# leosampaio/sketchformer

Hardware: AMD Instinct MI355X
Metric: stroke-tokens/sec training step, d_model=128 L=200 B=128, 1/2/4/8 GPU (higher is better)
Workload: dtype f32; 1 GPU; cfg2: sketch-transformer-tf2 4L/8H/d128/dff512 L=200 V=1004 C=345 dropout=0.1, fwd+bwd+Adam(WarmupDecay); global_batch=128, per_gpu_batch=128, seq_len=200, parallelism=dp1, hip_graph=0, dense_gemm_arithmetic=fp32 operands split exactly into 3 bf16 pieces, 6 product...

## Files before the change

### sketchformer_amd/csrc/skf_model_bwd.hip

```cpp
#include "skf_model_internal.h"

namespace skf_model_detail {
namespace {

template <typename F>
int with_ready_event(SkfModel* M, bool want, hipEvent_t* ready, F call) {
  hipEvent_t e = (want && may_park(M)) ? M->sched.take_event() : nullptr;
  bool rode = false;
  const int rc = with_tail_event(M, e, &rode, call);
  *ready = rode ? e : nullptr;
  return rc;
}

int ffn_bwd(SkfModel* M, const DenseP& f1, const DenseP& f2, const float* x_in, const float* h, const float* dy,
            float* dh, float* dx_acc, int rows, hipStream_t s, const void* hbits, const void* image_t) {
  if (M->ctx.ffn_fused) {
    SKF_TRY(dense_wgrad(M, f2, h, f2.in, dy, f2.out, rows, s));
    SKF_TRY(M->sched.before_write(M, dh, s));
    SKF_TRY(M->sched.before_write(M, dx_acc, s));
    const int* blocks = M->ctx.live_blocks(rows, 16);
    hipEvent_t ready = nullptr;
    SKF_TRY(with_ready_event(M, M->sched.holding(), &ready, [&] {
      return skf_ffn_fused_bwd_f32(rows, M->cfg.d_model, M->cfg.dff, dy, image_t, hbits, dh, dx_acc, 1, blocks, blocks ? 16 : 0,
                                   M->cfg.gemm_precision, s);
// ... 113 lines not shown
  SKF_TRY(skf_target_live_len(M->at<long long>(P.tar), Le, B, Ld, M->at<int>(P.live_len), s));
  SKF_TRY(skf_row_blocks_build(M->at<int>(P.live_len), B, Ld, 16, M->at<int>(P.live16), s));
  SKF_TRY(skf_row_blocks_build(M->at<int>(P.live_len), B, Ld, 32, M->at<int>(P.live32), s));
  M->ctx.lists_built = true;
  return SKF_OK;
}

}

int run_backward(SkfModel* M, hipStream_t s) {
  M->ctx.begin_backward();
  M->sched.begin_backward();
  M->red.begin_step();
  const SkfConfig& c = M->cfg;
  const Layout& L = M->lay;
  const Plan& P = M->plan;
  const int B = c.batch, Le = c.seq_len, Ld = c.seq_len - 1, d = c.d_model, H = c.num_heads, dh = d / H;
  const int Me = B * Le, Md = B * Ld, N = c.num_layers;
  const float rate = c.dropout_rate;
  const long long* inp = M->at<long long>(P.inp);
  const long long* tar = M->at<long long>(P.tar);
  const unsigned char* emask = M->at<unsigned char>(P.enc_mask);
  const unsigned char* dmask = M->at<unsigned char>(P.dec_mask);
  float* G = M->at<float>(P.gA);
  float* G2 = M->at<float>(P.gB);
  float* dO = M->at<float>(P.do_);
  float* dpre = M->at<float>(P.dpre);
  float* demb = M->at<float>(P.demb);
  int layer_no = 0;

  const bool bott = has_bott(c), cls = has_cls(c), recon = do_recon(c);
  float* enc_out = M->at<float>(P.enc[N - 1].x2);
  const float* pre = bott ? M->at<float>(P.pre) : enc_out;
  if (recon) {
  if (!M->ctx.lists_built) SKF_TRY(build_row_lists(M, s));
  if (M->ctx.lists_built) M->ctx.set_live(Md, M->at<int>(P.live_len), 16, M->at<int>(P.live16), 32, M->at<int>(P.live32));
  M->ctx.lists_built = false;
  const float* dlog = M->at<float>(P.logits);
  SKF_TRY(dense_wgrad(M, L.out, M->at<float>(P.dec[N - 1].out3), d, dlog, L.out.out, Md, s));
  {
    hipEvent_t ready = nullptr;
    SKF_TRY(with_ready_event(M, true, &ready, [&] { return dense_dgrad(M, L.out, dlog, L.out.out, Md, G, d, 0, nullptr, 0, s); }));
    SKF_TRY(M->sched.issue(M, s, ready));
  }
  const unsigned char* cross_mask = c.blind_decoder_mask ? nullptr : emask;
  for (int i = N - 1; i >= 0; --i, ++layer_no) {
    const DecLayerP& w = L.dec[i];
    const DecAct& a = P.dec[i];
    const Plan::GradSet& gs = P.gs[layer_no % P.n_gs];
    float* dy3 = M->at<float>(gs.dy[0]); float* dy2 = M->at<float>(gs.dy[1]); float* dy1 = M->at<float>(gs.dy[2]);
    float* dqkv = M->at<float>(gs.dqkv); float* dkv2 = M->at<float>(gs.dkv2); float* dq2 = M->at<float>(gs.dq2);
    SKF_TRY(ffn_ln_bwd(M, w.ln3, w.f1, w.f2, G, M->at<float>(a.z3), M->at<float>(a.st3), M->at<float>(a.out2), M->at<float>(a.h), dy3,
                       M->at<float>(gs.dh), G2, Md, rate, site_dec(N, i, 2), s, hbits_of(M, a.hbits, Md), M->at<char>(a.img[1])));
    SKF_TRY(ln_oproj_bwd(M, w.ln2, w.mha2.o, G2, M->at<float>(a.z2), M->at<float>(a.st2), M->at<float>(a.o2), G, dy2, dO, Md, rate,
                         site_dec(N, i, 1), s, M->at<char>(a.img_o2)));
    const float* kv2 = M->at<float>(a.kv2);
    SKF_TRY(M->sched.before_write(M, dq2, s));
    SKF_TRY(M->sched.before_write(M, dkv2, s));
    const int* qlive = M->ctx.live_lengths(Md);
    SKF_TRY(skf_attention_bwd_ordered(M->at<float>(a.q2), d, kv2, 2 * d, kv2 + d, 2 * d, M->at<float>(a.o2), d, dO, d,
                                      M->at<float>(a.astats2), cross_mask, Le, 0, B, H, Ld, Le, dh, dq2, d, dkv2, 2 * d,
                                      dkv2 + d, 2 * d, M->cfg.gemm_precision, qlive, M->ctx.order, s));
    SKF_TRY(dense_wgrad(M, w.mha2.q, M->at<float>(a.out1), d, dq2, d, Md, s));
    const bool lead = row_owner_takes_ln(M, w.ln1, ln_oproj_partial_bytes(M, Md), Md, &w.mha1.o, &w.mha2.q);
    if (!lead) SKF_TRY(dense_dgrad(M, w.mha2.q, dq2, d, Md, G, d, 1, nullptr, 0, s));
    SKF_TRY(dense_wgrad(M, w.mha2.kv, pre, L.E, dkv2, 2 * d, Me, s));
    if (i == 0) {
      SKF_TRY(M->sched.before_read(M, dpre, s));
      SKF_TRY(dense_dgrad(M, w.mha2.kv, dkv2, 2 * d, Me, dpre, L.E, i != N - 1, nullptr, 0, s));
    } else SKF_TRY(dense_dgrad_deferred(M, w.mha2.kv, dkv2, 2 * d, Me, dpre, L.E, i != N - 1, s));
    SKF_TRY(ln_oproj_bwd(M, w.ln1, w.mha1.o, G, M->at<float>(a.z1), M->at<float>(a.st1), M->at<float>(a.o1), G2, dy1, dO, Md, rate,
                         site_dec(N, i, 0), s, M->at<char>(a.img_o1), lead ? dq2 : nullptr, lead ? M->at<char>(a.img_q2t) : nullptr));
    const float* qkv = M->at<float>(a.qkv);
    SKF_TRY(M->sched.before_write(M, dqkv, s));
    SKF_TRY(skf_attention_bwd_ordered(qkv, 3 * d, qkv + d, 3 * d, qkv + 2 * d, 3 * d, M->at<float>(a.o1), d, dO, d,
                                      M->at<float>(a.astats1), dmask, Ld, 1, B, H, Ld, Ld, dh, dqkv, 3 * d, dqkv + d, 3 * d,
                                      dqkv + 2 * d, 3 * d, M->cfg.gemm_precision, qlive, M->ctx.order, s));
    SKF_TRY(dense_wgrad(M, w.mha1.qkv, M->at<float>(a.x_in), d, dqkv, 3 * d, Md, s));
    const bool hold = M->ctx.ffn_fused && i > 0;
    hipEvent_t ready = nullptr;
    SKF_TRY(with_ready_event(M, !hold, &ready, [&] { return dense_dgrad(M, w.mha1.qkv, dqkv, 3 * d, Md, G2, d, 1, nullptr, 0, s); }));
    float* t = G; G = G2; G2 = t;
    if (hold) SKF_TRY(M->sched.hold(M, s));
    else SKF_TRY(M->sched.issue(M, s, ready));
  }
  M->ctx.clear_live();
  hipEvent_t dec_emb_done = nullptr;
  if (c.continuous) {
    SKF_TRY(skf_embed_continuous_bwd(M->at<float>(P.tar), Le, B, Ld, G, d, M->G(L.dec_embd.w), M->G(L.dec_embd.b), rate,
                                     site_dec_embed(N), M->state, M->at<char>(P.small_ws), P.small_ws_bytes, s));
  } else {
    if (P.emb_sort_bytes) {
      SKF_TRY(with_ready_event(M, M->n_buckets == 2, &dec_emb_done, [&] {
        return skf_embed_bwd_sorted(M->at<char>(P.emb_sort[1]), B, Ld, G, c.vocab_size, d, M->G(L.dec_emb), rate, site_dec_embed(N), M->state, s);
      }));
    } else {
      SKF_HIP(hipMemsetAsync(M->G(L.dec_emb), 0, (size_t)c.vocab_size * d * sizeof(float), s));
      SKF_TRY(skf_embed_bwd(tar, Le, B, Ld, G, c.vocab_size, d, M->G(L.dec_emb), rate, site_dec_embed(N), M->state, s));
    }
  }
  if (M->n_buckets == 2) SKF_TRY(flush_wgrads(M, s, 0, false, true, dec_emb_done));
  SKF_TRY(M->sched.before_read(M, dpre, s));
  }
  const int E = L.E, Ua = L.Ua, U = c.lowerdim, NB = c.class_buffer_layers;
  hipEvent_t bott_ready = nullptr;
  if (bott) {
    const bool defer_sums = M->sched.side && Ua <= 4096;
    float* xp1 = M->at<float>(P.bott_part);
    float* xp2 = xp1 + (size_t)B * Le;
    float* pvp = xp2 + (size_t)B * Le;
    if (recon && defer_sums) {
      SKF_TRY(skf_expander_bwd_partials(dpre, M->at<float>(P.emb), M->P(L.exp_w), B, Le, E, demb, 0, xp1, xp2, s));
      SKF_TRY(colsum_desc(M, xp1, B, Le, M->G(L.exp_w)));
      SKF_TRY(colsum_desc(M, xp2, B, Le, M->G(L.exp_b)));
    } else if (recon)
      SKF_TRY(skf_expander_bwd(dpre, M->at<float>(P.emb), M->P(L.exp_w), B, Le, E, demb, 0, M->G(L.exp_w), M->G(L.exp_b),
                               M->at<char>(P.small_ws), P.small_ws_bytes, s));
    const int acc_emb = recon ? 1 : 0;
    const float* dcls = M->at<float>(P.cls_logits);
    if (cls && NB == 0) {
      SKF_TRY(dense_wgrad(M, L.cls, M->at<float>(P.emb), E, dcls, c.n_classes, B, s));
      SKF_TRY(dense_dgrad(M, L.cls, dcls, c.n_classes, B, demb, E, acc_emb, nullptr, 0, s));
    } else if (cls) {
      float* dz = M->at<float>(P.dcb[0]);
      float* dz2 = M->at<float>(P.dcb[1]);
      SKF_TRY(M->sched.before_write(M, dz, s));
      SKF_TRY(dense_wgrad(M, L.cls, M->at<float>(P.cb_f[NB - 1]), U, dcls, c.n_classes, B, s));
      SKF_TRY(dense_dgrad(M, L.cls, dcls, c.n_classes, B, dz, U, 0, M->at<float>(P.cb_h[NB - 1]), U, s));
      for (int i = NB - 1; i >= 0; --i) {
        SKF_TRY(skf_dropout(dz, dz, (size_t)B * U, c.class_dropout, site_class(N, i), M->state, s));
        const float* in = i == 0 ? M->at<float>(P.emb) : M->at<float>(P.cb_f[i - 1]);
        const int in_w = i == 0 ? E : U;
        SKF_TRY(dense_wgrad(M, L.cbuf[i], in, in_w, dz, U, B, s));
        if (i == 0) {
          SKF_TRY(dense_dgrad(M, L.cbuf[0], dz, U, B, demb, E, acc_emb, nullptr, 0, s));
        } else {
          SKF_TRY(M->sched.before_write(M, dz2, s));
          SKF_TRY(dense_dgrad(M, L.cbuf[i], dz, U, B, dz2, U, 0, M->at<float>(P.cb_h[i - 1]), U, s));
          float* t = dz; dz = dz2; dz2 = t;
        }
      }
    }
    const float* dpool = demb;
    if (c.attn_version == 2) {
      SKF_TRY(M->sched.before_write(M, M->at<float>(P.dpooled), s));
      SKF_TRY(dense_wgrad(M, L.bott_e, M->at<float>(P.pooled), d, demb, U, B, s));
      SKF_TRY(dense_dgrad(M, L.bott_e, demb, U, B, M->at<float>(P.dpooled), d, 0, nullptr, 0, s));
      dpool = M->at<float>(P.dpooled);
    }
    SKF_TRY(M->sched.before_write(M, G, s));
    if (defer_sums) {
      SKF_TRY(skf_pool_bwd_partials(M->at<float>(P.u), M->P(L.bott_v), enc_out, M->at<float>(P.pool_a), dpool, B, Le, Ua, d, G, pvp, s));
      SKF_TRY(colsum_desc(M, pvp, B, Ua, M->G(L.bott_v)));
    } else
    SKF_TRY(skf_pool_bwd(M->at<float>(P.u), M->P(L.bott_v), enc_out, M->at<float>(P.pool_a), dpool, B, Le, Ua, d,
                         G, M->G(L.bott_v), M->at<char>(P.small_ws), P.small_ws_bytes, s));
    SKF_TRY(dense_wgrad(M, L.bott_w, enc_out, d, M->at<float>(P.u), Ua, Me, s));
    SKF_TRY(with_ready_event(M, true, &bott_ready, [&] { return dense_dgrad(M, L.bott_w, M->at<float>(P.u), Ua, Me, G, d, 1, nullptr, 0, s); }));
  } else {
    float* spare = (G == M->at<float>(P.gA)) ? M->at<float>(P.gB) : M->at<float>(P.gA);
    G = dpre; G2 = spare;
  }
  SKF_TRY(M->sched.issue(M, s, bott_ready));
  for (int i = N - 1; i >= 0; --i, ++layer_no) {
    const EncLayerP& w = L.enc[i];
    const EncAct& a = P.enc[i];
    const Plan::GradSet& gs = P.gs[layer_no % P.n_gs];
    float* dy2 = M->at<float>(gs.dy[0]); float* dy1 = M->at<float>(gs.dy[1]);
    float* dqkv = M->at<float>(gs.dqkv);
    SKF_TRY(ffn_ln_bwd(M, w.ln2, w.f1, w.f2, G, M->at<float>(a.z2), M->at<float>(a.st2), M->at<float>(a.x1), M->at<float>(a.h), dy2,
                       M->at<float>(gs.dh), G2, Me, rate, site_enc(i, 1), s, hbits_of(M, a.hbits, Me), M->at<char>(a.img[1])));
    if (i == 0) SKF_TRY(M->sched.issue(M, s, M->ctx.last_ready));
    M->ctx.last_ready = nullptr;
    {
      hipEvent_t ready = nullptr;
      SKF_TRY(with_ready_event(M, i == 0, &ready, [&] {
        return ln_oproj_bwd(M, w.ln1, w.mha.o, G2, M->at<float>(a.z1), M->at<float>(a.st1), M->at<float>(a.o), G, dy1, dO, Me, rate,
                            site_enc(i, 0), s, M->at<char>(a.img_o));
      }));
      if (i == 0) SKF_TRY(M->sched.issue(M, s, ready));
    }
    const float* qkv = M->at<float>(a.qkv);
// ... 57 lines not shown
```

### sketchformer_amd/csrc/skf_model_fwd.hip

```cpp
#include "skf_model_internal.h"

namespace skf_model_detail {

int classify_fwd(SkfModel* M, bool training, hipStream_t s) {
  const SkfConfig& c = M->cfg;
  const Layout& L = M->lay;
  const Plan& P = M->plan;
  const float* fc = M->at<float>(P.emb);
  for (int i = 0; i < c.class_buffer_layers; ++i) {
    float* h = M->at<float>(P.cb_h[i]);
    float* fdrop = M->at<float>(P.cb_f[i]);
    SKF_TRY(dense_fwd(M, L.cbuf[i], fc, c.batch, h, 1, s));
    const float r = training ? c.class_dropout : 0.f;
    SKF_TRY(skf_dropout(h, fdrop, (size_t)c.batch * c.lowerdim, r, site_class(c.num_layers, i), M->state, s));
    fc = fdrop;
  }
  return dense_fwd(M, L.cls, fc, c.batch, M->at<float>(P.cls_logits), 0, s);
}

namespace {
bool ffn_fused_on(const SkfModel* M) {
  const SkfConfig& c = M->cfg;
  return !(M->flags & SKF_MODEL_FFN_LAUNCHES) && skf_ffn_fused_supported(c.batch * c.seq_len, c.d_model, c.dff, c.gemm_precision) &&
         skf_ffn_image_bytes(c.d_model, c.dff, c.gemm_precision) > 0;
}
int build_ffn_images(SkfModel* M, bool with_backward, bool encoder_only, hipStream_t s) {
  const SkfConfig& c = M->cfg;
  const Layout& L = M->lay;
  const Plan& P = M->plan;
  const int d = c.d_model, F = c.dff;
  const size_t half = skf_ffn_image_bytes(d, F, c.gemm_precision) / 2;
  std::vector<const float*> src; std::vector<int> ld, tr, K, N; std::vector<void*> img;
  auto one = [&](const DenseP& w, int t, int k, int n, char* im) {
    src.push_back(M->P(w.w)); ld.push_back(w.ld); tr.push_back(t); K.push_back(k); N.push_back(n); img.push_back(im);
  };
  auto ffn = [&](const DenseP& f1, const DenseP& f2, const size_t (&im)[2]) {
    one(f1, 0, d, F, M->at<char>(im[0])); one(f2, 0, F, d, M->at<char>(im[0]) + half);
    if (with_backward) { one(f2, 1, d, F, M->at<char>(im[1])); one(f1, 1, F, d, M->at<char>(im[1]) + half); }
  };
  const bool dec = !encoder_only && do_recon(c);
  for (int i = 0; i < c.num_layers; ++i) {
    ffn(L.enc[i].f1, L.enc[i].f2, P.enc[i].img);
    if (i > 0) one(L.enc[i].mha.qkv, 0, d, 3 * d, M->at<char>(P.enc[i].img_qkv));
    one(L.enc[i].mha.o, 0, d, d, M->at<char>(P.enc[i].img_of));
    if (with_backward) one(L.enc[i].mha.o, 1, d, d, M->at<char>(P.enc[i].img_o));
  }
  if (dec)
    for (int i = 0; i < c.num_layers; ++i) {
      ffn(L.dec[i].f1, L.dec[i].f2, P.dec[i].img);
      if (i > 0) one(L.dec[i].mha1.qkv, 0, d, 3 * d, M->at<char>(P.dec[i].img_qkv));
      one(L.dec[i].mha2.o, 0, d, d, M->at<char>(P.dec[i].img_o2f));
      one(L.dec[i].mha1.o, 0, d, d, M->at<char>(P.dec[i].img_o1f)); one(L.dec[i].mha2.q, 0, d, d, M->at<char>(P.dec[i].img_q2));
      if (with_backward) { one(L.dec[i].mha1.o, 1, d, d, M->at<char>(P.dec[i].img_o1)); one(L.dec[i].mha2.o, 1, d, d, M->at<char>(P.dec[i].img_o2)); }
// ... 92 lines not shown
    SKF_TRY(skf_embed_continuous_fwd(inpf, Le, B, Le, M->P(L.enc_embd.w), M->P(L.enc_embd.b), d, M->pos,
                                     M->at<float>(P.enc[0].x_in), rate, site_enc_embed(), M->state, s));
  else
    SKF_TRY(skf_embed_fwd(inp, Le, B, Le, M->P(L.enc_emb), c.vocab_size, d, M->pos, M->at<float>(P.enc[0].x_in), rate,
                          site_enc_embed(), M->state, s));
  bool enc_qkv_done = false;
  for (int i = 0; i < N; ++i) {
    const EncLayerP& w = L.enc[i];
    const EncAct& a = P.enc[i];
    float* x = M->at<float>(a.x_in);
    float* qkv = M->at<float>(a.qkv);
    if (!enc_qkv_done) SKF_TRY(dense_fwd(M, w.mha.qkv, x, Me, qkv, 0, s));
    if (i == 0 && images_ready) SKF_HIP(hipStreamWaitEvent(s, masks_ready, 0));
    SKF_TRY(skf_attention_fwd_ordered(qkv, 3 * d, qkv + d, 3 * d, qkv + 2 * d, 3 * d, emask, Le, 0, B, H, Le, Le, dh,
                                      M->at<float>(a.o), d, M->at<float>(a.astats), M->cfg.gemm_precision, order, s));
    const bool has_next = i + 1 < N;
    if (i == 0 && images_ready) SKF_HIP(hipStreamWaitEvent(s, images_ready, 0));
    SKF_TRY(attn_tail_ffn_fwd(M, w.mha.o, w.ln1, M->at<float>(a.o), x, M->at<float>(a.z1), M->at<float>(a.x1), M->at<float>(a.st1),
                              site_enc(i, 0), M->at<char>(a.img_of), w.f1, w.f2, w.ln2, M->at<float>(a.h), hbits_of(M, a.hbits, Me),
                              M->at<char>(a.img[0]), M->at<float>(a.z2), M->at<float>(a.x2), M->at<float>(a.st2), site_enc(i, 1), Me, rate, s,
                              has_next ? &L.enc[i + 1].mha.qkv : nullptr, has_next ? M->at<char>(P.enc[i + 1].img_qkv) : nullptr,
                              has_next ? M->at<float>(P.enc[i + 1].qkv) : nullptr, &enc_qkv_done));
  }
  float* enc_out = M->at<float>(P.enc[N - 1].x2);
  const int E = L.E, Ua = L.Ua;
  const bool bott = has_bott(c), cls = has_cls(c), recon = do_recon(c);
  if (bott) {
    SKF_TRY(dense_fwd(M, L.bott_w, enc_out, Me, M->at<float>(P.u), 2, s));
    SKF_TRY(skf_pool_fwd(M->at<float>(P.u), M->P(L.bott_v), enc_out, B, Le, Ua, d, M->at<float>(P.pool_a),
                         M->at<float>(c.attn_version == 2 ? P.pooled : P.emb), s));
    if (c.attn_version == 2)
      SKF_TRY(dense_fwd(M, L.bott_e, M->at<float>(P.pooled), B, M->at<float>(P.emb), 0, s));
  }
  if (cls) SKF_TRY(classify_fwd(M, training, s));
  if (encoder_only || !recon) {
    if (encoder_only || !with_loss) {
      if (!cls) return SKF_OK;
      return skf_softmax_ce(M->at<float>(P.cls_logits), c.n_classes, B, c.n_classes, M->at<long long>(P.labels), 1, 1, 0, 0, 0.f,
                            M->at<float>(P.cls_loss), M->at<float>(P.cls_hit), M->at<float>(P.cls_probs), 0, s);
    }
  }
  float* pre = bott ? M->at<float>(P.pre) : enc_out;
  hipEvent_t dec_in_ready = nullptr;
  bool dec_in_recorded = false;
  if (recon && M->sched.side) {
    M->sched.rewind_events();
    dec_in_ready = M->sched.take_event();
    SKF_CHECK_ARG(dec_in_ready, "event allocation failed");
  }
  if (recon && bott) {
    SKF_TRY(with_tail_event(M, dec_in_ready, &dec_in_recorded,
                            [&] { return skf_expander_fwd(M->at<float>(P.emb), M->P(L.exp_w), M->P(L.exp_b), B, Le, E, pre, s); }));
  }

  if (recon) {
  if (c.continuous)
    SKF_TRY(skf_embed_continuous_fwd(tarf, Le, B, Ld, M->P(L.dec_embd.w), M->P(L.dec_embd.b), d, M->pos,
                                     M->at<float>(P.dec[0].x_in), rate, site_dec_embed(N), M->state, s));
  else
    SKF_TRY(skf_embed_fwd(tar, Le, B, Ld, M->P(L.dec_emb), c.vocab_size, d, M->pos, M->at<float>(P.dec[0].x_in), rate,
                          site_dec_embed(N), M->state, s));
  const unsigned char* cross_mask = c.blind_decoder_mask ? nullptr : emask;
  hipEvent_t kv_done = nullptr, kv_first = nullptr;
  if (M->sched.side) {
    kv_done = M->sched.take_event();
    kv_first = N > 1 ? M->sched.take_event() : kv_done;
    SKF_CHECK_ARG(dec_in_ready && kv_done && kv_first, "event allocation failed");
    if (!dec_in_recorded) SKF_HIP(hipEventRecord(dec_in_ready, s));
    SKF_HIP(hipStreamWaitEvent(M->sched.side, dec_in_ready, 0));
    for (int i = 0; i < N; ++i) {
      SKF_TRY(dense_fwd(M, L.dec[i].mha2.kv, pre, Me, M->at<float>(P.dec[i].kv2), 0, M->sched.side));
      if (i == 0 && kv_first != kv_done) SKF_HIP(hipEventRecord(kv_first, M->sched.side));
    }
    SKF_HIP(hipEventRecord(kv_done, M->sched.side));
  }
  bool dec_qkv_done = false;
  for (int i = 0; i < N; ++i) {
    const DecLayerP& w = L.dec[i];
    const DecAct& a = P.dec[i];
    float* x = M->at<float>(a.x_in);
    float* qkv = M->at<float>(a.qkv);
    if (!dec_qkv_done) SKF_TRY(dense_fwd(M, w.mha1.qkv, x, Md, qkv, 0, s));
    SKF_TRY(skf_attention_fwd_ordered(qkv, 3 * d, qkv + d, 3 * d, qkv + 2 * d, 3 * d, dmask, Ld, 1, B, H, Ld, Ld, dh,
                                      M->at<float>(a.o1), d, M->at<float>(a.astats1), M->cfg.gemm_precision, order, s));
    const bool tail_proj = M->ctx.ffn_fused && w.mha1.o.in == d && w.mha1.o.out == d && chains(M, w.mha2.q) && w.mha2.q.out == d &&
                           w.ln1.b == w.ln1.g + (size_t)d;
    if (tail_proj) {
      SkfFfnBlockFwd tb{};
      tb.struct_size = sizeof(SkfFfnBlockFwd); tb.M = Md; tb.d = d; tb.dff = c.dff; tb.precision = c.gemm_precision;
      tb.x = M->at<float>(a.o1); tb.rate = rate; tb.step_state = M->state;
      tb.pre_image = M->at<char>(a.img_o1f); tb.pre_bias = M->P(w.mha1.o.b); tb.pre_residual = x; tb.pre_gamma = M->P(w.ln1.g); tb.pre_beta = M->P(w.ln1.b);
      tb.pre_z = M->at<float>(a.z1); tb.pre_out = M->at<float>(a.out1); tb.pre_stats = M->at<float>(a.st1); tb.pre_site = site_dec(N, i, 0);
      tb.proj_image = M->at<char>(a.img_q2); tb.proj_bias = M->P(w.mha2.q.b); tb.proj_out = M->at<float>(a.q2); tb.proj_n = d;
      SKF_TRY(skf_ffn_block_fwd_f32(&tb, s));
    } else {
      SKF_TRY(dense_ln_fwd(M, w.mha1.o, M->at<float>(a.o1), Md, x, M->at<float>(a.z1), w.ln1, M->at<float>(a.out1), M->at<float>(a.st1),
                           rate, site_dec(N, i, 0), s));
      SKF_TRY(dense_fwd(M, w.mha2.q, M->at<float>(a.out1), Md, M->at<float>(a.q2), 0, s));
    }
    float* kv2 = M->at<float>(a.kv2);
    if (!kv_done) SKF_TRY(dense_fwd(M, w.mha2.kv, pre, Me, kv2, 0, s));
    else if (i == 0) SKF_HIP(hipStreamWaitEvent(s, kv_first, 0));
    else if (i == 1) SKF_HIP(hipStreamWaitEvent(s, kv_done, 0));
    SKF_TRY(skf_attention_fwd_ordered(M->at<float>(a.q2), d, kv2, 2 * d, kv2 + d, 2 * d, cross_mask, Le, 0, B, H, Ld, Le, dh,
                                      M->at<float>(a.o2), d, M->at<float>(a.astats2), M->cfg.gemm_precision, order, s));
    const bool has_next = i + 1 < N;
    SKF_TRY(attn_tail_ffn_fwd(M, w.mha2.o, w.ln2, M->at<float>(a.o2), M->at<float>(a.out1), M->at<float>(a.z2), M->at<float>(a.out2),
                              M->at<float>(a.st2), site_dec(N, i, 1), M->at<char>(a.img_o2f), w.f1, w.f2, w.ln3, M->at<float>(a.h),
                              hbits_of(M, a.hbits, Md), M->at<char>(a.img[0]), M->at<float>(a.z3), M->at<float>(a.out3), M->at<float>(a.st3),
                              site_dec(N, i, 2), Md, rate, s, has_next ? &L.dec[i + 1].mha1.qkv : nullptr,
                              has_next ? M->at<char>(P.dec[i + 1].img_qkv) : nullptr, has_next ? M->at<float>(P.dec[i + 1].qkv) : nullptr,
                              &dec_qkv_done));
  }
  SKF_TRY(dense_fwd(M, L.out, M->at<float>(P.dec[N - 1].out3), Md, M->at<float>(P.logits), 0, s));
  }

  const long long* labels = M->at<long long>(P.labels);
  if (with_loss) {
    const float* recon_scalar = nullptr;
    if (recon) {
      if (c.continuous) {
        SKF_TRY(skf_continuous_loss(M->at<float>(P.logits), tarf, Le, Ld, 1, Md, c.recon_weight, M->at<float>(P.recon_loss),
                                    M->at<float>(P.recon_hit), M->at<float>(P.row_mask), M->at<float>(P.cont_scal), 1, s));
        recon_scalar = M->at<float>(P.cont_scal) + 3;
      } else {
        SKF_TRY(skf_softmax_ce(M->at<float>(P.logits), c.vocab_size, Md, c.vocab_size, tar, Le, Ld, 1, 1,
                               c.recon_weight / (float)Md, M->at<float>(P.recon_loss), M->at<float>(P.recon_hit), nullptr, 1, s));
      }
    }
    if (cls)
      SKF_TRY(skf_softmax_ce(M->at<float>(P.cls_logits), c.n_classes, B, c.n_classes, labels, 1, 1, 0, 0,
                             c.class_weight / (float)B, M->at<float>(P.cls_loss), M->at<float>(P.cls_hit),
                             M->at<float>(P.cls_probs), 1, s));
    SKF_TRY(skf_metrics_update(M->at<float>(P.recon_loss), M->at<float>(P.recon_hit), recon ? Md : 0, c.recon_weight,
                               M->at<float>(P.cls_loss), M->at<float>(P.cls_hit), cls ? B : 0, c.class_weight, recon_scalar,
                               M->metrics, s));
  } else if (cls) {
    SKF_TRY(skf_softmax_ce(M->at<float>(P.cls_logits), c.n_classes, B, c.n_classes, labels, 1, 1, 0, 0, 0.f,
                           M->at<float>(P.cls_loss), M->at<float>(P.cls_hit), M->at<float>(P.cls_probs), 0, s));
  }
  return SKF_OK;
}

}
```

### sketchformer_amd/csrc/skf_model_internal.h

```cpp
#pragma once
#include <stdarg.h>
#include <stdlib.h>
#include <string.h>
#include <string>
#include <vector>
#include <map>
#include <algorithm>
#include "skf_common.h"
#include "skf_attention_params.h"
#include "skf_decode_fused.h"

namespace skf_model_detail {

struct DenseP { size_t w, b; int in, out, ld; };
struct LnP { size_t g, b; };
struct SelfMhaP { DenseP qkv, o; };
struct CrossMhaP { DenseP q, kv, o; };
struct EncLayerP { SelfMhaP mha; DenseP f1, f2; LnP ln1, ln2; };
struct DecLayerP { SelfMhaP mha1; CrossMhaP mha2; DenseP f1, f2; LnP ln1, ln2, ln3; };

inline bool has_bott(const SkfConfig& c) { return c.lowerdim > 0; }
inline bool has_cls(const SkfConfig& c) { return c.lowerdim > 0 && c.do_classification != 0; }
inline bool do_recon(const SkfConfig& c) { return c.do_reconstruction != 0; }

struct Layout {
  size_t total = 0;
  size_t enc_emb = 0, dec_emb = 0;
  DenseP enc_embd{}, dec_embd{};
  std::vector<EncLayerP> enc;
  std::vector<DecLayerP> dec;
  DenseP bott_w{};
  size_t bott_v = 0;
  DenseP bott_e{};
  std::vector<DenseP> cbuf;
  size_t dec_off = 0;
  int E = 0, Ua = 0;
  DenseP cls{}, out{};
  size_t exp_w = 0, exp_b = 0;
  std::vector<SkfParamEntry> entries;
};
// ... 64 lines not shown
  size_t live_len = 0, live1 = 0, live64 = 0;
  size_t emb_sort[2] = {0, 0}, emb_sort_bytes = 0;
  std::map<size_t, Img16> img;
};

struct ReduceBatch {
  std::vector<SkfReduceDesc> descs;
  bool descs_uploaded = false;
  size_t slab_cursor = 0, desc_cursor = 0, ln_cursor = 0;
  int reduce_blocks = 0;
  size_t phase_desc_begin = 0;
  bool side_used = false;

  void begin_step();
  void reset();
  int add(const SkfReduceDesc& d, int blocks);
  float* take_ln_partial(SkfModel* M);
  float* take_slab(SkfModel* M, size_t bytes, size_t queued);
  size_t begin() const { return phase_desc_begin; }
  size_t end() const { return desc_cursor; }
  int blocks() const { return reduce_blocks; }
  void end_phase(bool final);
};

struct SideSched {
  hipStream_t side = nullptr;
  hipEvent_t fork_event = nullptr, join_event = nullptr;
  std::vector<hipEvent_t> events;
  size_t next_event = 0;
  struct SideEvent { hipEvent_t e; long seq; };
  long side_seq = 0, side_waited = 0;
  std::map<const void*, SideEvent> pending_readers;
  std::map<const void*, SideEvent> pending_writers;
  struct Queued { DenseP w; const float* x; int ldx; const float* dy; int lddy; int rows; int kind = 0; float* dx = nullptr; int lddx = 0; int accumulate = 0; const int* blocks32 = nullptr; };
  std::vector<Queued> wq;
  std::vector<Queued> wq_held;

  int create(bool captured);
  void destroy();
  hipEvent_t take_event();
  void rewind_events() { next_event = 0; }
  void begin_backward() { wq.clear(); wq_held.clear(); pending_readers.clear(); pending_writers.clear(); rewind_events(); }
  void queue_wgrad(const DenseP& w, const float* x, int ldx, const float* dy, int lddy, int rows, const int* blocks32) { wq.push_back(Queued{w, x, ldx, dy, lddy, rows, 0, nullptr, 0, 0, blocks32}); }
  void queue_dgrad(const DenseP& w, const float* dy, int lddy, int rows, float* dx, int lddx, int accumulate) { wq.push_back(Queued{w, nullptr, 0, dy, lddy, rows, 1, dx, lddx, accumulate}); }
  bool holding() const { return !wq_held.empty(); }
  int hold(SkfModel* M, hipStream_t s);
  int issue(SkfModel* M, hipStream_t s, hipEvent_t ready_recorded = nullptr, bool on_main = false);
  int issue_held(SkfModel* M, hipStream_t s, hipEvent_t ready_recorded = nullptr);
  int before_write(SkfModel* M, const void* buf, hipStream_t s) { return wait_side(M, false, buf, s); }
  int before_read(SkfModel* M, const void* buf, hipStream_t s) { return wait_side(M, true, buf, s); }
  int wait_side(SkfModel* M, bool writers, const void* buf, hipStream_t s);
  int join(hipStream_t s);
  bool fork_into_capture(hipStream_t s) { return hipEventRecord(fork_event, s) == hipSuccess && hipStreamWaitEvent(side, fork_event, 0) == hipSuccess; }
  bool join_capture(hipStream_t s) { return hipEventRecord(join_event, side) == hipSuccess && hipStreamWaitEvent(s, join_event, 0) == hipSuccess; }
};

struct StepCtx {
  bool lists_set = false;
  int live_rows = 0;
  const int* live_len = nullptr;
  struct LiveList { int granule; const int* blocks; } lists[2] = {};
  const int* order = nullptr;
  hipEvent_t pre_ready = nullptr, masks_ready = nullptr;
  bool lists_built = false;
  bool masks_staged = false;
  bool ffn_fused = false;
  hipEvent_t last_ready = nullptr;

  void reset() { *this = StepCtx(); }
  void begin_backward() { clear_live(); last_ready = nullptr; }
  void set_live(int rows, const int* len, int g0, const int* b0, int g1, const int* b1) { lists_set = true; live_rows = rows; live_len = len; lists[0] = {g0, b0}; lists[1] = {g1, b1}; }
  void clear_live() { lists_set = false; live_rows = 0; live_len = nullptr; lists[0] = lists[1] = LiveList{}; }
  bool live(int rows) const { return lists_set && rows == live_rows; }
  const int* live_lengths(int rows) const { return live(rows) ? live_len : nullptr; }
  const int* live_blocks(int rows, int granule) const {
    return !live(rows) ? nullptr : lists[0].granule == granule ? lists[0].blocks : lists[1].granule == granule ? lists[1].blocks : nullptr;
  }
};

}

struct SkfModel {
  SkfConfig cfg;
  uint32_t flags = 0;
  bool no_ln_fuse = false, no_relu_bits = false;
  skf_model_detail::StepCtx ctx;
  skf_model_detail::Layout lay;
  skf_model_detail::Plan plan;
  skf_model_detail::Plan16 p16;
  bool bf16 = false;
  float *params = nullptr, *grads = nullptr, *m = nullptr, *v = nullptr, *metrics = nullptr;
  const float* pos = nullptr;
  char* ws = nullptr;
  void* state = nullptr;
  hipGraphExec_t g_fb = nullptr, g_opt = nullptr, g_dec = nullptr;
  long long dec_dyn_host[2] = {0, 0};
  std::vector<int> dec_stream_host;
  std::vector<int> dec_pfx_len_host;
  float g_opt_scale = 0.f;
// ... 22 lines not shown
  } while (0)

namespace skf_model_detail {

extern thread_local int g_capturing;

inline unsigned site_enc_embed() { return 0; }
inline unsigned site_enc(int layer, int j) { return 1 + 2 * layer + j; }
inline unsigned site_dec_embed(int N) { return 1 + 2 * N; }
inline unsigned site_class(int N, int i) { return 2 + 5 * N + i; }
inline unsigned site_dec(int N, int layer, int j) { return 2 + 2 * N + 3 * layer + j; }

inline bool may_park(const SkfModel* M, bool needs_side = true) { return !g_capturing && (M->sched.side || !needs_side); }
template <typename F>
int with_tail_event(SkfModel* M, hipEvent_t e, bool* rode, F call, bool needs_side = true) {
  SkfTailScope scope(may_park(M, needs_side) ? e : nullptr);
  const int rc = call();
  *rode = scope.attached();
  return rc;
}

Layout build_layout(const SkfConfig& c);
bool decode_areas_ok(const DecodeAreas& A, size_t plan_bytes);
Plan build_plan(const SkfConfig& c);
Plan16 build_plan16(const SkfConfig& c, const Layout& L);

int dense_fwd(SkfModel* M, const DenseP& w, const float* x, int rows, float* y, int act, hipStream_t s);
int dense_ln_fwd(SkfModel* M, const DenseP& w, const float* a, int rows, const float* x, float* z, const LnP& ln, float* out,
                 float* stats, float rate, unsigned site, hipStream_t s);
void* hbits_of(SkfModel* M, size_t off, int rows);
int dense_fwd_relu_bits(SkfModel* M, const DenseP& w, const float* x, int rows, float* y, void* bits, hipStream_t s);
int dense_fwd_ld(SkfModel* M, const DenseP& w, const float* x, int ldx, int rows, float* y, int ldy, int act, hipStream_t s);
int dense_wgrad(SkfModel* M, const DenseP& w, const float* x, int ldx, const float* dy, int lddy, int rows, hipStream_t s);
int flush_wgrads(SkfModel* M, hipStream_t s, int bucket, bool final, bool issue_queued = true, hipEvent_t main_here = nullptr);
int dense_dgrad(SkfModel* M, const DenseP& w, const float* dy, int lddy, int rows, float* dx, int lddx, int accumulate,
                const float* relu_src, int ld_relu, hipStream_t s, const void* relu_bits = nullptr);
int dense_dgrad_deferred(SkfModel* M, const DenseP& w, const float* dy, int lddy, int rows, float* dx, int lddx, int accumulate,
                         hipStream_t s);

int classify_fwd(SkfModel* M, bool training, hipStream_t s);
int forward_preamble(SkfModel* M, bool with_backward, bool encoder_only, hipStream_t s, hipEvent_t masks_ready = nullptr);
int run_forward(SkfModel* M, bool training, bool with_loss, hipStream_t s, bool encoder_only = false);
int run_backward(SkfModel* M, hipStream_t s);
int issue_embed_sorts(SkfModel* M, hipStream_t s);

struct BeamOut { long long* tokens; float* scores; int* lengths; };
struct DecodeRequest {
  const float* embedding = nullptr;
  const int* expected_len_host = nullptr;
  int n_valid = 0;
  long long sos = 0, eos = 0;
  int max_steps = 0;
  void* out = nullptr;
  int* out_len_host = nullptr;
  float* attn = nullptr;
  const SkfSampling* smp = nullptr;
  const int* stream_ids_host = nullptr;
  const SkfBeam* bm = nullptr;
  const BeamOut* bm_out = nullptr;
  const SkfPrefix* pfx = nullptr;
};
int run_decode(SkfModel* M, const DecodeRequest& rq, hipStream_t s);

void register_buffers16(SkfModel* M);
int ensure_cast_table16(SkfModel* M, hipStream_t s);
int run_forward16(SkfModel* M, bool training, bool with_loss, hipStream_t s, bool encoder_only = false);
int run_backward16(SkfModel* M, hipStream_t s);
int issue_embed_sorts16(SkfModel* M, hipStream_t s);
}
```

### sketchformer_amd/csrc/skf_model_sched.hip

```cpp
#include "skf_model_internal.h"

namespace skf_model_detail {

int dense_fwd(SkfModel* M, const DenseP& w, const float* x, int rows, float* y, int act, hipStream_t s) {
  return skf_gemm_f32(1, 0, rows, w.out, w.in, x, w.in, M->P(w.w), w.ld, y, w.out, M->P(w.b), act, nullptr, 0, 0, 1,
                      nullptr, 0, nullptr, 0, M->cfg.gemm_precision, s);
}
int dense_ln_fwd(SkfModel* M, const DenseP& w, const float* a, int rows, const float* x, float* z, const LnP& ln, float* out,
                 float* stats, float rate, unsigned site, hipStream_t s) {
  if (!M->no_ln_fuse && skf_gemm_ln_residual_supported(rows, w.out, w.in, M->cfg.gemm_precision)) {
    const int rc = skf_gemm_ln_residual_f32(rows, w.out, w.in, a, w.in, M->P(w.w), w.ld, M->P(w.b), x, M->P(ln.g), M->P(ln.b), z, out, stats,
                                            rate, site, M->state, M->cfg.gemm_precision, s);
    if (rc != SKF_EUNSUPPORTED) return rc;
    M->no_ln_fuse = true;
  }
  SKF_TRY(dense_fwd(M, w, a, rows, z, 0, s));
  return skf_layernorm_residual_fwd(x, z, M->P(ln.g), M->P(ln.b), out, stats, rows, w.out, rate, site, M->state, s);
}
void* hbits_of(SkfModel* M, size_t off, int rows) {
  if (M->ctx.ffn_fused) return M->at<char>(off);
  if (M->no_relu_bits || !skf_gemm_relu_bits_bytes(rows, M->cfg.dff, M->cfg.d_model, M->cfg.gemm_precision)) return nullptr;
  return M->at<char>(off);
}
int dense_fwd_relu_bits(SkfModel* M, const DenseP& w, const float* x, int rows, float* y, void* bits, hipStream_t s) {
// ... 62 lines not shown
int SideSched::hold(SkfModel* M, hipStream_t s) {
  if (!wq_held.empty()) SKF_TRY(issue(M, s));
  wq_held.swap(wq);
  return SKF_OK;
}
int SideSched::issue(SkfModel* M, hipStream_t s, hipEvent_t ready_recorded, bool on_main) {
  SkfTailScope shield(nullptr);
  SKF_TRY(issue_held(M, s));
  if (wq.empty()) return SKF_OK;
  std::vector<Queued> group;
  group.swap(wq);
  hipStream_t ws = on_main ? s : side;
  hipEvent_t ready = nullptr, done = nullptr;
  if (!on_main) {
    ready = ready_recorded ? ready_recorded : take_event(); done = take_event();
    SKF_CHECK_ARG(ready && done, "event allocation failed");
    if (!ready_recorded) SKF_HIP(hipEventRecord(ready, s));
    SKF_HIP(hipStreamWaitEvent(side, ready, 0));
  }
  hipEvent_t dgrad_done = nullptr;
  for (const auto& q : group) {
    if (q.kind != 1) continue;
    const DenseP& w = q.w;
    SKF_TRY(skf_gemm_f32(1, 1, q.rows, w.in, w.out, q.dy, q.lddy, M->P(w.w), w.ld, q.dx, q.lddx, nullptr, 0, nullptr, 0,
                         q.accumulate, 1, nullptr, 0, nullptr, 0, M->cfg.gemm_precision, ws));
    if (!dgrad_done && !on_main) { dgrad_done = take_event(); SKF_CHECK_ARG(dgrad_done, "event allocation failed"); }
  }
  long dgrad_seq = 0;
  if (dgrad_done) { SKF_HIP(hipEventRecord(dgrad_done, side)); dgrad_seq = ++side_seq; }
  std::vector<SkfWgradProblem> probs;
  std::vector<const Queued*> prob_q;
  for (const auto& q : group) {
    const DenseP& w = q.w;
    if (q.kind == 1) continue;
    if ((double)w.in * w.out * q.rows <= 33554432.0) {
      SKF_TRY(dense_wgrad_on(M, w, q.x, q.ldx, q.dy, q.lddy, q.rows, ws));
      continue;
    }
    const int splits = skf_gemm_default_splits(w.in, w.out, q.rows);
    const size_t bytes = (skf_gemm_workspace_bytes(w.in, w.out, q.rows, splits, 1) + 255) & ~(size_t)255;
    SkfWgradProblem pr{};
    pr.A = q.x; pr.B = q.dy; pr.slab = M->red.take_slab(M, bytes, probs.size()); pr.slab_bytes = bytes;
    if (!pr.slab) return SKF_EINVAL;
    pr.row_blocks = q.blocks32; pr.row_block_rows = 32;
    pr.M = w.in; pr.N = w.out; pr.K = q.rows; pr.lda = q.ldx; pr.ldb = q.lddy; pr.splits = splits; pr.with_bias_grad = 1;
    probs.push_back(pr); prob_q.push_back(&q);
  }
  bool small = true;
  for (const auto& pr : probs) small = small && 2.0 * pr.M * pr.N * pr.K < 4e9;
  const size_t gmax = small ? 8 : 1;
  for (size_t b0 = 0; b0 < probs.size(); b0 += gmax) {
    const int nb = (int)std::min<size_t>(gmax, probs.size() - b0);
    SKF_TRY(skf_gemm_wgrad_partial_group(probs.data() + b0, nb, M->cfg.gemm_precision, ws));
  }
  for (size_t i = 0; i < probs.size(); ++i) {
    const DenseP& w = prob_q[i]->w;
    SkfReduceDesc d;
    d.slab = probs[i].slab; d.C = M->G(w.w); d.bias_grad = M->G(w.b); d.splits = probs[i].splits_used; d.M = w.in; d.N = w.out; d.ldc = w.ld;
    d.block_begin = M->red.blocks(); d.pad = 0;
    SKF_TRY(M->red.add(d, skf_splitk_reduce_blocks(w.in, w.out)));
  }
  M->red.side_used = true;
  if (on_main) return SKF_OK;
  SKF_HIP(hipEventRecord(done, side));
  const long done_seq = ++side_seq;
  for (const auto& q : group) {
    pending_readers[q.dy] = SideEvent{done, done_seq};
    if (q.x) pending_readers[q.x] = SideEvent{done, done_seq};
    if (q.kind == 1) pending_writers[q.dx] = SideEvent{dgrad_done, dgrad_seq};
  }
  return SKF_OK;
}
int SideSched::join(hipStream_t s) {
  hipEvent_t e = take_event();
  SKF_CHECK_ARG(e, "event allocation failed");
  SKF_HIP(hipEventRecord(e, side));
  SKF_HIP(hipStreamWaitEvent(s, e, 0));
  pending_readers.clear();
  pending_writers.clear();
  side_waited = side_seq;
  return SKF_OK;
}
int dense_wgrad(SkfModel* M, const DenseP& w, const float* x, int ldx, const float* dy, int lddy, int rows, hipStream_t s) {
  if (!M->sched.side) return dense_wgrad_on(M, w, x, ldx, dy, lddy, rows, s);
  M->sched.queue_wgrad(w, x, ldx, dy, lddy, rows, M->ctx.live_blocks(rows, 32));
  return SKF_OK;
}
int flush_wgrads(SkfModel* M, hipStream_t s, int bucket, bool final, bool issue_queued, hipEvent_t main_here) {
  if (issue_queued) SKF_TRY(M->sched.issue(M, s));
  const size_t begin = M->red.begin(), end = M->red.end();
  hipStream_t ready_on = s;
  bool bucket_recorded = false;
  hipStream_t side = M->sched.side;
  if (side && M->red.side_used && end > begin) {
    if (!M->red.descs_uploaded) {
      SKF_HIP(hipMemcpy(M->at<SkfReduceDesc>(M->plan.descs) + begin, M->red.descs.data() + begin,
                        (end - begin) * sizeof(SkfReduceDesc), hipMemcpyHostToDevice));
      if (final) M->red.descs_uploaded = true;
    }
    if (final) {
      SKF_TRY(M->sched.join(s));
      SKF_TRY(with_tail_event(M, bucket >= 0 ? M->bucket_ready[bucket] : nullptr, &bucket_recorded, [&] {
        return skf_splitk_reduce_batch(M->at<SkfReduceDesc>(M->plan.descs) + begin, (int)(end - begin), M->red.blocks(), s);
      }));
    } else {
      hipEvent_t em = main_here ? main_here : M->sched.take_event();
      SKF_CHECK_ARG(em, "event allocation failed");
      if (!main_here) SKF_HIP(hipEventRecord(em, s));
      SKF_HIP(hipStreamWaitEvent(side, em, 0));
      SKF_TRY(skf_splitk_reduce_batch(M->at<SkfReduceDesc>(M->plan.descs) + begin, (int)(end - begin), M->red.blocks(), side));
      ready_on = side;
    }
  }
  if (bucket >= 0 && M->bucket_ready[bucket] && !bucket_recorded) SKF_HIP(hipEventRecord(M->bucket_ready[bucket], ready_on));
  M->red.end_phase(final);
  return SKF_OK;
}
int dense_dgrad(SkfModel* M, const DenseP& w, const float* dy, int lddy, int rows, float* dx, int lddx, int accumulate,
                const float* relu_src, int ld_relu, hipStream_t s, const void* relu_bits) {
  SKF_TRY(M->sched.before_write(M, dx, s));
  const int* blocks = M->ctx.live_blocks(rows, 16);
  if (relu_bits)
    return skf_gemm_f32_bits(1, 1, rows, w.in, w.out, dy, lddy, M->P(w.w), w.ld, dx, lddx, nullptr, 0, nullptr, 0,
                             accumulate, 1, nullptr, 0, nullptr, 0, M->cfg.gemm_precision, blocks, 16, nullptr, relu_bits, s);
  return skf_gemm_f32_rows(1, 1, rows, w.in, w.out, dy, lddy, M->P(w.w), w.ld, dx, lddx, nullptr, 0, relu_src, ld_relu,
                           accumulate, 1, nullptr, 0, nullptr, 0, M->cfg.gemm_precision, blocks, 16, s);
}

int dense_dgrad_deferred(SkfModel* M, const DenseP& w, const float* dy, int lddy, int rows, float* dx, int lddx, int accumulate,
                         hipStream_t s) {
  if (!M->sched.side) return dense_dgrad(M, w, dy, lddy, rows, dx, lddx, accumulate, nullptr, 0, s);
  M->sched.queue_dgrad(w, dy, lddy, rows, dx, lddx, accumulate);
  return SKF_OK;
}

void ReduceBatch::begin_step() {
  side_used = false;
  slab_cursor = 0; desc_cursor = 0; reduce_blocks = 0; phase_desc_begin = 0; ln_cursor = 0;
}
void ReduceBatch::reset() {
  descs.clear(); descs_uploaded = false;
  slab_cursor = 0; desc_cursor = 0; ln_cursor = 0; reduce_blocks = 0; phase_desc_begin = 0;
// ... 36 lines not shown
```

Baseline: 7.441 million stroke-tokens/sec.

## Move classifier head and decoder embedding backward onto side stream

The classifier forward and its cross-entropy loss now run on the side stream alongside the decoder K/V projections, and the metrics update is deferred into the backward pass. The sorted decoder-embedding backward becomes a generic queued launch issued on the side stream after the last decoder layer, so it overlaps with the bottleneck/encoder backward on the main stream. A spare gradient buffer (gC) is swapped in so the main stream does not overwrite the embedding's input while the side stream still reads it. This adds ordering assumptions between streams (metrics reading the side-written class loss, and the reduce skipping its main-stream wait), which is a correctness risk.

```diff
diff --git a/sketchformer_amd/csrc/skf_model_bwd.hip b/sketchformer_amd/csrc/skf_model_bwd.hip
--- a/sketchformer_amd/csrc/skf_model_bwd.hip
+++ b/sketchformer_amd/csrc/skf_model_bwd.hip
@@ -169,6 +169,7 @@
   const bool bott = has_bott(c), cls = has_cls(c), recon = do_recon(c);
   float* enc_out = M->at<float>(P.enc[N - 1].x2);
   const float* pre = bott ? M->at<float>(P.pre) : enc_out;
+  const bool dec_emb_on_side = recon && M->sched.side && !c.continuous && P.emb_sort_bytes;
   if (recon) {
   if (!M->ctx.lists_built) SKF_TRY(build_row_lists(M, s));
   if (M->ctx.lists_built) M->ctx.set_live(Md, M->at<int>(P.live_len), 16, M->at<int>(P.live16), 32, M->at<int>(P.live32));
@@ -218,25 +219,34 @@
     hipEvent_t ready = nullptr;
     SKF_TRY(with_ready_event(M, !hold, &ready, [&] { return dense_dgrad(M, w.mha1.qkv, dqkv, 3 * d, Md, G2, d, 1, nullptr, 0, s); }));
     float* t = G; G = G2; G2 = t;
+    if (i == 0 && dec_emb_on_side) {
+      const float* dx0 = G;
+      char* sorted = M->at<char>(P.emb_sort[1]);
+      float* dtable = M->G(L.dec_emb);
+      const int V = c.vocab_size;
+      M->sched.queue_launch(dx0, [M, sorted, dtable, dx0, B, Ld, V, d, rate, N](hipStream_t on) {
+        return skf_embed_bwd_sorted(sorted, B, Ld, dx0, V, d, dtable, rate, site_dec_embed(N), M->state, on);
+      });
+    }
     if (hold) SKF_TRY(M->sched.hold(M, s));
     else SKF_TRY(M->sched.issue(M, s, ready));
   }
   M->ctx.clear_live();
-  hipEvent_t dec_emb_done = nullptr;
+  if (M->ctx.metrics_deferred) {
+    M->ctx.metrics_deferred = false;
+    SKF_TRY(metrics_update(M, M->sched.side));
+  }
   if (c.continuous) {
     SKF_TRY(skf_embed_continuous_bwd(M->at<float>(P.tar), Le, B, Ld, G, d, M->G(L.dec_embd.w), M->G(L.dec_embd.b), rate,
                                      site_dec_embed(N), M->state, M->at<char>(P.small_ws), P.small_ws_bytes, s));
+  } else if (dec_emb_on_side) {
+  } else if (P.emb_sort_bytes) {
+    SKF_TRY(skf_embed_bwd_sorted(M->at<char>(P.emb_sort[1]), B, Ld, G, c.vocab_size, d, M->G(L.dec_emb), rate, site_dec_embed(N), M->state, s));
   } else {
-    if (P.emb_sort_bytes) {
-      SKF_TRY(with_ready_event(M, M->n_buckets == 2, &dec_emb_done, [&] {
-        return skf_embed_bwd_sorted(M->at<char>(P.emb_sort[1]), B, Ld, G, c.vocab_size, d, M->G(L.dec_emb), rate, site_dec_embed(N), M->state, s);
-      }));
-    } else {
-      SKF_HIP(hipMemsetAsync(M->G(L.dec_emb), 0, (size_t)c.vocab_size * d * sizeof(float), s));
-      SKF_TRY(skf_embed_bwd(tar, Le, B, Ld, G, c.vocab_size, d, M->G(L.dec_emb), rate, site_dec_embed(N), M->state, s));
-    }
-  }
-  if (M->n_buckets == 2) SKF_TRY(flush_wgrads(M, s, 0, false, true, dec_emb_done));
+    SKF_HIP(hipMemsetAsync(M->G(L.dec_emb), 0, (size_t)c.vocab_size * d * sizeof(float), s));
+    SKF_TRY(skf_embed_bwd(tar, Le, B, Ld, G, c.vocab_size, d, M->G(L.dec_emb), rate, site_dec_embed(N), M->state, s));
+  }
+  if (M->n_buckets == 2) SKF_TRY(flush_wgrads(M, s, 0, false, true, dec_emb_on_side));
   SKF_TRY(M->sched.before_read(M, dpre, s));
   }
   const int E = L.E, Ua = L.Ua, U = c.lowerdim, NB = c.class_buffer_layers;
@@ -285,6 +295,7 @@
       SKF_TRY(dense_dgrad(M, L.bott_e, demb, U, B, M->at<float>(P.dpooled), d, 0, nullptr, 0, s));
       dpool = M->at<float>(P.dpooled);
     }
+    if (dec_emb_on_side) { G = G2; G2 = M->at<float>(P.gC); }
     SKF_TRY(M->sched.before_write(M, G, s));
     if (defer_sums) {
       SKF_TRY(skf_pool_bwd_partials(M->at<float>(P.u), M->P(L.bott_v), enc_out, M->at<float>(P.pool_a), dpool, B, Le, Ua, d, G, pvp, s));
diff --git a/sketchformer_amd/csrc/skf_model_fwd.hip b/sketchformer_amd/csrc/skf_model_fwd.hip
--- a/sketchformer_amd/csrc/skf_model_fwd.hip
+++ b/sketchformer_amd/csrc/skf_model_fwd.hip
@@ -18,7 +18,24 @@
   return dense_fwd(M, L.cls, fc, c.batch, M->at<float>(P.cls_logits), 0, s);
 }
 
+int metrics_update(SkfModel* M, hipStream_t s) {
+  const SkfConfig& c = M->cfg;
+  const Plan& P = M->plan;
+  const bool recon = do_recon(c);
+  const float* recon_scalar = recon && c.continuous ? M->at<float>(P.cont_scal) + 3 : nullptr;
+  return skf_metrics_update(M->at<float>(P.recon_loss), M->at<float>(P.recon_hit), recon ? c.batch * (c.seq_len - 1) : 0, c.recon_weight,
+                            M->at<float>(P.cls_loss), M->at<float>(P.cls_hit), has_cls(c) ? c.batch : 0, c.class_weight, recon_scalar,
+                            M->metrics, s);
+}
+
 namespace {
+int class_ce_with_grad(SkfModel* M, hipStream_t s) {
+  const SkfConfig& c = M->cfg;
+  const Plan& P = M->plan;
+  return skf_softmax_ce(M->at<float>(P.cls_logits), c.n_classes, c.batch, c.n_classes, M->at<long long>(P.labels), 1, 1, 0, 0,
+                        c.class_weight / (float)c.batch, M->at<float>(P.cls_loss), M->at<float>(P.cls_hit), M->at<float>(P.cls_probs), 1, s);
+}
+
 bool ffn_fused_on(const SkfModel* M) {
   const SkfConfig& c = M->cfg;
   return !(M->flags & SKF_MODEL_FFN_LAUNCHES) && skf_ffn_fused_supported(c.batch * c.seq_len, c.d_model, c.dff, c.gemm_precision) &&
@@ -177,7 +194,8 @@
     if (c.attn_version == 2)
       SKF_TRY(dense_fwd(M, L.bott_e, M->at<float>(P.pooled), B, M->at<float>(P.emb), 0, s));
   }
-  if (cls) SKF_TRY(classify_fwd(M, training, s));
+  const bool heads_on_side = with_loss && recon && M->sched.side;
+  if (cls && !heads_on_side) SKF_TRY(classify_fwd(M, training, s));
   if (encoder_only || !recon) {
     if (encoder_only || !with_loss) {
       if (!cls) return SKF_OK;
@@ -213,6 +231,10 @@
     SKF_CHECK_ARG(dec_in_ready && kv_done && kv_first, "event allocation failed");
     if (!dec_in_recorded) SKF_HIP(hipEventRecord(dec_in_ready, s));
     SKF_HIP(hipStreamWaitEvent(M->sched.side, dec_in_ready, 0));
+    if (cls && heads_on_side) {
+      SKF_TRY(classify_fwd(M, training, M->sched.side));
+      SKF_TRY(class_ce_with_grad(M, M->sched.side));
+    }
     for (int i = 0; i < N; ++i) {
       SKF_TRY(dense_fwd(M, L.dec[i].mha2.kv, pre, Me, M->at<float>(P.dec[i].kv2), 0, M->sched.side));
       if (i == 0 && kv_first != kv_done) SKF_HIP(hipEventRecord(kv_first, M->sched.side));
@@ -262,24 +284,18 @@
 
   const long long* labels = M->at<long long>(P.labels);
   if (with_loss) {
-    const float* recon_scalar = nullptr;
     if (recon) {
       if (c.continuous) {
         SKF_TRY(skf_continuous_loss(M->at<float>(P.logits), tarf, Le, Ld, 1, Md, c.recon_weight, M->at<float>(P.recon_loss),
                                     M->at<float>(P.recon_hit), M->at<float>(P.row_mask), M->at<float>(P.cont_scal), 1, s));
-        recon_scalar = M->at<float>(P.cont_scal) + 3;
       } else {
         SKF_TRY(skf_softmax_ce(M->at<float>(P.logits), c.vocab_size, Md, c.vocab_size, tar, Le, Ld, 1, 1,
                                c.recon_weight / (float)Md, M->at<float>(P.recon_loss), M->at<float>(P.recon_hit), nullptr, 1, s));
       }
     }
-    if (cls)
-      SKF_TRY(skf_softmax_ce(M->at<float>(P.cls_logits), c.n_classes, B, c.n_classes, labels, 1, 1, 0, 0,
-                             c.class_weight / (float)B, M->at<float>(P.cls_loss), M->at<float>(P.cls_hit),
-                             M->at<float>(P.cls_probs), 1, s));
-    SKF_TRY(skf_metrics_update(M->at<float>(P.recon_loss), M->at<float>(P.recon_hit), recon ? Md : 0, c.recon_weight,
-                               M->at<float>(P.cls_loss), M->at<float>(P.cls_hit), cls ? B : 0, c.class_weight, recon_scalar,
-                               M->metrics, s));
+    if (cls && !heads_on_side) SKF_TRY(class_ce_with_grad(M, s));
+    if (heads_on_side) M->ctx.metrics_deferred = true;
+    else SKF_TRY(metrics_update(M, s));
   } else if (cls) {
     SKF_TRY(skf_softmax_ce(M->at<float>(P.cls_logits), c.n_classes, B, c.n_classes, labels, 1, 1, 0, 0, 0.f,
                            M->at<float>(P.cls_loss), M->at<float>(P.cls_hit), M->at<float>(P.cls_probs), 0, s));
diff --git a/sketchformer_amd/csrc/skf_model_internal.h b/sketchformer_amd/csrc/skf_model_internal.h
--- a/sketchformer_amd/csrc/skf_model_internal.h
+++ b/sketchformer_amd/csrc/skf_model_internal.h
@@ -6,6 +6,7 @@
 #include <vector>
 #include <map>
 #include <algorithm>
+#include <functional>
 #include "skf_common.h"
 #include "skf_attention_params.h"
 #include "skf_decode_fused.h"
@@ -136,7 +137,7 @@
   long side_seq = 0, side_waited = 0;
   std::map<const void*, SideEvent> pending_readers;
   std::map<const void*, SideEvent> pending_writers;
-  struct Queued { DenseP w; const float* x; int ldx; const float* dy; int lddy; int rows; int kind = 0; float* dx = nullptr; int lddx = 0; int accumulate = 0; const int* blocks32 = nullptr; };
+  struct Queued { DenseP w; const float* x; int ldx; const float* dy; int lddy; int rows; int kind = 0; float* dx = nullptr; int lddx = 0; int accumulate = 0; const int* blocks32 = nullptr; std::function<int(hipStream_t)> run; };
   std::vector<Queued> wq;
   std::vector<Queued> wq_held;
 
@@ -147,6 +148,7 @@
   void begin_backward() { wq.clear(); wq_held.clear(); pending_readers.clear(); pending_writers.clear(); rewind_events(); }
   void queue_wgrad(const DenseP& w, const float* x, int ldx, const float* dy, int lddy, int rows, const int* blocks32) { wq.push_back(Queued{w, x, ldx, dy, lddy, rows, 0, nullptr, 0, 0, blocks32}); }
   void queue_dgrad(const DenseP& w, const float* dy, int lddy, int rows, float* dx, int lddx, int accumulate) { wq.push_back(Queued{w, nullptr, 0, dy, lddy, rows, 1, dx, lddx, accumulate}); }
+  void queue_launch(const float* reads, std::function<int(hipStream_t)> run) { Queued q{}; q.dy = reads; q.kind = 2; q.run = std::move(run); wq.push_back(std::move(q)); }
   bool holding() const { return !wq_held.empty(); }
   int hold(SkfModel* M, hipStream_t s);
   int issue(SkfModel* M, hipStream_t s, hipEvent_t ready_recorded = nullptr, bool on_main = false);
@@ -169,6 +171,7 @@
   bool lists_built = false;
   bool masks_staged = false;
   bool ffn_fused = false;
+  bool metrics_deferred = false;
   hipEvent_t last_ready = nullptr;
 
   void reset() { *this = StepCtx(); }
@@ -257,13 +260,14 @@
 int dense_fwd_relu_bits(SkfModel* M, const DenseP& w, const float* x, int rows, float* y, void* bits, hipStream_t s);
 int dense_fwd_ld(SkfModel* M, const DenseP& w, const float* x, int ldx, int rows, float* y, int ldy, int act, hipStream_t s);
 int dense_wgrad(SkfModel* M, const DenseP& w, const float* x, int ldx, const float* dy, int lddy, int rows, hipStream_t s);
-int flush_wgrads(SkfModel* M, hipStream_t s, int bucket, bool final, bool issue_queued = true, hipEvent_t main_here = nullptr);
+int flush_wgrads(SkfModel* M, hipStream_t s, int bucket, bool final, bool issue_queued = true, bool side_behind_main = false);
 int dense_dgrad(SkfModel* M, const DenseP& w, const float* dy, int lddy, int rows, float* dx, int lddx, int accumulate,
                 const float* relu_src, int ld_relu, hipStream_t s, const void* relu_bits = nullptr);
 int dense_dgrad_deferred(SkfModel* M, const DenseP& w, const float* dy, int lddy, int rows, float* dx, int lddx, int accumulate,
                          hipStream_t s);
 
 int classify_fwd(SkfModel* M, bool training, hipStream_t s);
+int metrics_update(SkfModel* M, hipStream_t s);
 int forward_preamble(SkfModel* M, bool with_backward, bool encoder_only, hipStream_t s, hipEvent_t masks_ready = nullptr);
 int run_forward(SkfModel* M, bool training, bool with_loss, hipStream_t s, bool encoder_only = false);
 int run_backward(SkfModel* M, hipStream_t s);
diff --git a/sketchformer_amd/csrc/skf_model_sched.hip b/sketchformer_amd/csrc/skf_model_sched.hip
--- a/sketchformer_amd/csrc/skf_model_sched.hip
+++ b/sketchformer_amd/csrc/skf_model_sched.hip
@@ -118,7 +118,7 @@
   std::vector<const Queued*> prob_q;
   for (const auto& q : group) {
     const DenseP& w = q.w;
-    if (q.kind == 1) continue;
+    if (q.kind != 0) continue;
     if ((double)w.in * w.out * q.rows <= 33554432.0) {
       SKF_TRY(dense_wgrad_on(M, w, q.x, q.ldx, q.dy, q.lddy, q.rows, ws));
       continue;
@@ -147,6 +147,8 @@
     SKF_TRY(M->red.add(d, skf_splitk_reduce_blocks(w.in, w.out)));
   }
   M->red.side_used = true;
+  for (const auto& q : group)
+    if (q.kind == 2) SKF_TRY(q.run(ws));
   if (on_main) return SKF_OK;
   SKF_HIP(hipEventRecord(done, side));
   const long done_seq = ++side_seq;
@@ -172,7 +174,7 @@
   M->sched.queue_wgrad(w, x, ldx, dy, lddy, rows, M->ctx.live_blocks(rows, 32));
   return SKF_OK;
 }
-int flush_wgrads(SkfModel* M, hipStream_t s, int bucket, bool final, bool issue_queued, hipEvent_t main_here) {
+int flush_wgrads(SkfModel* M, hipStream_t s, int bucket, bool final, bool issue_queued, bool side_behind_main) {
   if (issue_queued) SKF_TRY(M->sched.issue(M, s));
   const size_t begin = M->red.begin(), end = M->red.end();
   hipStream_t ready_on = s;
@@ -190,10 +192,12 @@
         return skf_splitk_reduce_batch(M->at<SkfReduceDesc>(M->plan.descs) + begin, (int)(end - begin), M->red.blocks(), s);
       }));
     } else {
-      hipEvent_t em = main_here ? main_here : M->sched.take_event();
-      SKF_CHECK_ARG(em, "event allocation failed");
-      if (!main_here) SKF_HIP(hipEventRecord(em, s));
-      SKF_HIP(hipStreamWaitEvent(side, em, 0));
+      if (!side_behind_main) {
+        hipEvent_t em = M->sched.take_event();
+        SKF_CHECK_ARG(em, "event allocation failed");
+        SKF_HIP(hipEventRecord(em, s));
+        SKF_HIP(hipStreamWaitEvent(side, em, 0));
+      }
       SKF_TRY(skf_splitk_reduce_batch(M->at<SkfReduceDesc>(M->plan.descs) + begin, (int)(end - begin), M->red.blocks(), side));
       ready_on = side;
     }
```

Measured after the change: 7.519 million stroke-tokens/sec (median of 6 runs). +1.1%, better.
